# Manta-Network/Plonk-Prototype

Hardware: AMD Instinct MI355X
Metric: bls12_381_fr_ntt_butterflies_per_s (higher is better)
Workload: dtype u32x9 (29-bit limbs, Fr); 1 GPU; forward + inverse BLS12-381 Fr NTT, 2^20 points, device resident, natural order in/out, bit-exact vs oracle; log_n=20, parallelism=1 independent polynomial(s), one per GPU

## Files before the change

### include/plonk_mi355x.h

```cpp
#ifndef PLONK_MI355X_H
#define PLONK_MI355X_H

#include <stddef.h>
#include <stdint.h>

#ifdef __cplusplus
extern "C" {
#endif

typedef struct pm_ctx pm_ctx;
typedef struct pm_bases pm_bases;

typedef enum {
  PM_OK = 0,
  PM_ERR_BAD_ARG = -1,
  PM_ERR_DOMAIN_TOO_LARGE = -2,
  PM_ERR_OOM = -3,
  PM_ERR_HIP = -4,
  PM_ERR_NO_DEVICE = -5,
  PM_ERR_LENGTH = -6,
  PM_ERR_EXCHANGE = -7,
  PM_ERR_BUSY = -8,
  PM_ERR_POINT = -9
} pm_status;
// ... 411 lines not shown
int pm_profile_select(pm_ctx* ctx, const char* kernel_name);
int pm_profile_read(pm_ctx* ctx, char* buf, size_t cap);
int pm_test_field_op(pm_ctx* ctx, int op, const uint64_t* a, const uint64_t* b, uint64_t* out,
                     size_t n);
int pm_test_field_raw_op(pm_ctx* ctx, int field, int op, const uint32_t* in, uint32_t* out, size_t n);
int pm_test_g1_raw_op(pm_ctx* ctx, int op, const uint32_t* a, const uint32_t* b, uint32_t* out, size_t n);
int pm_test_glv_split(pm_ctx* ctx, const uint64_t* scalars, size_t n, uint32_t scalar_form, uint64_t* out);
int pm_test_host_glv_split(const uint64_t k[4], uint64_t out[4]);
int pm_test_jubjub_scalar_op(pm_ctx* ctx, int op, const uint64_t* a, const uint64_t* b, const uint64_t* c, uint64_t* out, size_t n);
int pm_test_host_jubjub_scalar_op(int op, const uint64_t* a, const uint64_t* b, const uint64_t* c, uint64_t* out, size_t n);
int pm_test_schnorr_stride(pm_ctx* ctx, size_t* stride);
int pm_test_cipher_stride(pm_ctx* ctx, size_t* stride);
int pm_test_cipher_digits(const uint64_t view_key[4], uint32_t scalar_form, int8_t digits[64]);
int pm_test_jubjub_msm_plan(size_t n, uint32_t batch, long window_bits, uint32_t num_cus, uint64_t out[8]);
int pm_test_jubjub_msm_digits(const uint64_t scalar[4], uint32_t c, int32_t* digits, uint32_t* n_digits);
int pm_test_host_field_op(int op, const uint64_t* a, const uint64_t* b, uint64_t* out, size_t n);
int pm_test_msm_sizing(size_t n, uint32_t batch, long window_bits, uint32_t table_window_bits, uint32_t num_cus,
                       uint64_t out[4]);
int pm_test_msm_plan(size_t n, uint32_t batch, long window_bits, uint32_t table_window_bits, uint32_t num_cus, long chunk,
                     long lb, uint32_t out[32], uint32_t* level_len);
int pm_test_ntt_plan(uint32_t log_n, uint32_t batch, long tile_log, long max_radix, long radix, uint32_t num_cus,
                     uint32_t out[20]);
int pm_test_ntt_step4_table(pm_ctx* ctx, uint32_t inverse, uint32_t S, uint32_t* out, size_t max_words, size_t* words);
int pm_test_ntt_exchange_map(uint32_t S, uint32_t LT, uint32_t ufast, uint32_t step, uint32_t tid, uint32_t out[12]);
int pm_test_wire_sort_plan(size_t n, size_t num_vars, uint32_t* passes, uint32_t* tiles, size_t* scratch_bytes);
int pm_test_host_naf(const uint64_t s[4], uint32_t rounds, int8_t* digits_msb_first, int* too_long);
int pm_test_msm_geometry(size_t n, long window_bits, uint32_t table_window_bits, uint32_t batch, uint32_t out[16],
                         uint32_t* part_of_bucket, uint32_t* first_bucket, uint32_t* width_bits);
int pm_test_plonk_linearise(size_t n, const uint64_t (*evaluations)[4], const uint64_t (*extras)[4],
                            const uint64_t (*challenges)[4], uint32_t selector_present_mask, uint64_t (*out_coeffs)[4],
                            uint32_t* out_roles, uint32_t* out_count, uint64_t out_r_z[4]);

#ifdef __cplusplus
}
#endif
#endif
```

### plonk-prototype_amd/_lib.py

```python
from __future__ import annotations

import ctypes as C
import os

_HERE = os.path.dirname(os.path.abspath(__file__))
LIB_PATH = os.environ.get("PM_LIB_PATH") or os.path.join(_HERE, "lib", "libplonk_mi355x.so")

u64p = C.POINTER(C.c_uint64)
u32p = C.POINTER(C.c_uint32)



class PermArgs(C.Structure):
    _fields_ = [("wires", C.c_void_p * 4), ("sigmas", C.c_void_p * 4), ("roots", C.c_void_p),
                ("beta", C.c_uint64 * 4), ("gamma", C.c_uint64 * 4), ("k", (C.c_uint64 * 4) * 3)]


class QuotientArgs(C.Structure):
    _fields_ = [("wires", C.c_void_p * 4), ("z", C.c_void_p), ("q_m", C.c_void_p), ("q_l", C.c_void_p),
                ("q_r", C.c_void_p), ("q_o", C.c_void_p), ("q_4", C.c_void_p), ("q_c", C.c_void_p),
                ("pi", C.c_void_p), ("sigmas", C.c_void_p * 4), ("l1", C.c_void_p), ("x", C.c_void_p),
                ("alpha", C.c_uint64 * 4), ("beta", C.c_uint64 * 4), ("gamma", C.c_uint64 * 4),
                ("k", (C.c_uint64 * 4) * 3), ("zh_inv", (C.c_uint64 * 4) * 4),
                ("q_arith", C.c_void_p), ("q_range", C.c_void_p), ("q_logic", C.c_void_p),
# ... 235 lines not shown
    "pm_test_comm_deadline": (C.c_int, [C.c_long, C.c_int, C.POINTER(C.c_int), C.POINTER(C.c_long), C.POINTER(C.c_int),
                                        C.POINTER(C.c_int), C.c_char_p, C.c_size_t]),
    "pm_keccak_f1600": (None, [C.c_char_p]),
    "pm_ntt_plan": (C.c_int, [C.c_uint32, u32p, u32p]),
    "pm_set_option": (C.c_int, [C.c_void_p, C.c_char_p, C.c_long]),
    "pm_profile_enable": (C.c_int, [C.c_void_p, C.c_int]),
    "pm_profile_select": (C.c_int, [C.c_void_p, C.c_char_p]),
    "pm_profile_read": (C.c_int, [C.c_void_p, C.c_char_p, C.c_size_t]),
    "pm_test_field_op": (C.c_int, [C.c_void_p, C.c_int, u64p, u64p, u64p, C.c_size_t]),
    "pm_test_field_raw_op": (C.c_int, [C.c_void_p, C.c_int, C.c_int, u32p, u32p, C.c_size_t]),
    "pm_test_g1_raw_op": (C.c_int, [C.c_void_p, C.c_int, u32p, u32p, u32p, C.c_size_t]),
    "pm_test_glv_split": (C.c_int, [C.c_void_p, u64p, C.c_size_t, C.c_uint32, u64p]),
    "pm_test_host_glv_split": (C.c_int, [u64p, u64p]),
    "pm_test_jubjub_scalar_op": (C.c_int, [C.c_void_p, C.c_int, u64p, u64p, u64p, u64p, C.c_size_t]),
    "pm_test_host_jubjub_scalar_op": (C.c_int, [C.c_int, u64p, u64p, u64p, u64p, C.c_size_t]),
    "pm_test_schnorr_stride": (C.c_int, [C.c_void_p, C.POINTER(C.c_size_t)]),
    "pm_test_cipher_stride": (C.c_int, [C.c_void_p, C.POINTER(C.c_size_t)]),
    "pm_test_cipher_digits": (C.c_int, [u64p, C.c_uint32, C.POINTER(C.c_int8)]),
    "pm_test_jubjub_msm_plan": (C.c_int, [C.c_size_t, C.c_uint32, C.c_long, C.c_uint32, u64p]),
    "pm_test_jubjub_msm_digits": (C.c_int, [u64p, C.c_uint32, C.POINTER(C.c_int32), u32p]),
    "pm_test_ntt_plan": (C.c_int, [C.c_uint32, C.c_uint32, C.c_long, C.c_long, C.c_long, C.c_uint32, C.POINTER(C.c_uint32)]),
    "pm_test_ntt_exchange_map": (C.c_int, [C.c_uint32] * 5 + [C.POINTER(C.c_uint32)]),
    "pm_test_ntt_step4_table": (C.c_int, [C.c_void_p, C.c_uint32, C.c_uint32, u32p, C.c_size_t, C.POINTER(C.c_size_t)]),
    "pm_test_wire_sort_plan": (C.c_int, [C.c_size_t, C.c_size_t, u32p, u32p, C.POINTER(C.c_size_t)]),
    "pm_test_host_naf": (C.c_int, [u64p, C.c_uint32, C.POINTER(C.c_int8), C.POINTER(C.c_int)]),
    "pm_test_msm_sizing": (C.c_int, [C.c_size_t, C.c_uint32, C.c_long, C.c_uint32, C.c_uint32, u64p]),
    "pm_test_msm_plan": (C.c_int, [C.c_size_t, C.c_uint32, C.c_long, C.c_uint32, C.c_uint32, C.c_long, C.c_long,
                                   u32p, u32p]),
    "pm_test_msm_geometry": (C.c_int, [C.c_size_t, C.c_long, C.c_uint32, C.c_uint32, C.POINTER(C.c_uint32),
                                      C.POINTER(C.c_uint32), C.POINTER(C.c_uint32), C.POINTER(C.c_uint32)]),
    "pm_test_plonk_linearise": (C.c_int, [C.c_size_t, u64p, u64p, u64p, C.c_uint32, u64p, u32p, u32p, u64p]),
}

PM_OK = 0
PM_ERR_BAD_ARG = -1
PM_ERR_DOMAIN_TOO_LARGE = -2
PM_ERR_OOM = -3
PM_ERR_HIP = -4
PM_ERR_NO_DEVICE = -5
PM_ERR_LENGTH = -6
PM_ERR_EXCHANGE = -7
PM_ERR_BUSY = -8
PM_ERR_POINT = -9

G1_CHECK_SUBGROUP = 1
G1_POINTS_IN_SUBGROUP = 1
# ... 78 lines not shown
```

### plonk-prototype_amd/csrc/api.hip

```cpp
#include <hip/hip_runtime.h>

#include <cstdio>
#include <cstdlib>
#include <cstring>

#include "context.h"
#include "field_inv.hip.h"
#include "fields.hip.h"
#include "host_field.h"
#include "jubjub_msm_plan.h"

namespace pm {

int set_err(pm_ctx* ctx, int code, const std::string& msg) {
  if (ctx) ctx->err = msg;
  return code;
}

int raise_lds_limit(pm_ctx* ctx, const void* fn, size_t bytes) {
  static std::mutex mu;
  static std::map<std::pair<int, const void*>, size_t> limit;
  std::lock_guard<std::mutex> lock(mu);
  size_t& have = limit[{ctx->device, fn}];
  if (bytes <= have) return PM_OK;
// ... 101 lines not shown
  int count = 0;
  if (hipGetDeviceCount(&count) != hipSuccess || count <= 0 || device_id < 0 || device_id >= count)
    return PM_ERR_NO_DEVICE;
  hipDeviceProp_t prop;
  if (hipGetDeviceProperties(&prop, device_id) != hipSuccess) return PM_ERR_NO_DEVICE;
  if (strncmp(prop.gcnArchName, "gfx950", 6) != 0) return PM_ERR_NO_DEVICE;
  if (hipSetDevice(device_id) != hipSuccess) return PM_ERR_HIP;
  pm_ctx* ctx = new pm_ctx();
  ctx->device = device_id;
  ctx->marks_on = getenv("PM_HOST_MARKS") != nullptr;
  ctx->num_cus = prop.multiProcessorCount;
  if (hipStreamCreateWithFlags(&ctx->stream, hipStreamNonBlocking) != hipSuccess) {
    delete ctx;
    return PM_ERR_HIP;
  }
  *out = ctx;
  return PM_OK;
}

static void release_caches(pm_ctx* ctx, bool all) {
  for (int d = 0; d < 2; ++d) {
    for (auto& kv : ctx->step_tw[d]) (void)hipFree(kv.second);
    for (auto& kv : ctx->step4_tw[d]) (void)hipFree(kv.second);
    for (auto& kv : ctx->domain[d]) {
      (void)hipFree(kv.second.tw_hi);
      (void)hipFree(kv.second.tw_lo);
      (void)hipFree(kv.second.cs_hi);
      (void)hipFree(kv.second.cs_lo);
      for (void* t : kv.second.pass_tw) (void)hipFree(t);
    }
    ctx->step_tw[d].clear();
    ctx->step4_tw[d].clear();
    ctx->domain[d].clear();
  }
  for (DeviceBuffer* b : {&ctx->ntt_tmp[0], &ctx->ntt_tmp[1], &ctx->io_in, &ctx->io_out, &ctx->msm_ws, &ctx->msm_scalars,
                          &ctx->poly_ws, &ctx->poly_tab, &ctx->jj_msm_ws, &ctx->fr_sqrt_tab}) {
    if (b->ptr) (void)hipFree(b->ptr);
    b->ptr = nullptr;
    b->bytes = 0;
  }
  if (all && ctx->msm_ctl.ptr) (void)hipFree(ctx->msm_ctl.ptr);
}

extern "C" int pm_trim(pm_ctx* ctx, size_t* freed_bytes) {
  if (!ctx) return PM_ERR_BAD_ARG;
  std::lock_guard<std::mutex> lk(ctx->mu);
  if (ctx->calls_holding_tables > 0)
    return set_err(ctx, PM_ERR_BUSY, "pm_trim while a pm_fr_ntt_fourstep_dev call is in flight on this context");
  PM_HIP(ctx, hipSetDevice(ctx->device));
  PM_HIP(ctx, hipDeviceSynchronize());
  size_t free0 = 0, free1 = 0, total = 0;
  PM_HIP(ctx, hipMemGetInfo(&free0, &total));
  release_caches(ctx, false);
  PM_HIP(ctx, hipMemGetInfo(&free1, &total));
  if (freed_bytes) *freed_bytes = free1 > free0 ? free1 - free0 : 0;
// ... 240 lines not shown
```

### plonk-prototype_amd/csrc/context.h

```cpp
#pragma once
#include <hip/hip_runtime.h>

#include <cstdint>
#include <initializer_list>
#include <map>
#include <chrono>
#include <mutex>
#include <string>
#include <vector>

#include "../../include/plonk_mi355x.h"

#ifndef PM_NTT_STEP_PRIO_DEFAULT
#define PM_NTT_STEP_PRIO_DEFAULT 1
#endif

namespace pm {

class ExchangeWatch;
void exchange_watch_free(ExchangeWatch* w);

struct DeviceBuffer {
  void* ptr = nullptr;
  size_t bytes = 0;
// ... 6 lines not shown
  hipEvent_t ev = nullptr;
};

struct NttDomainTables {
  void* tw_hi = nullptr;
  void* tw_lo = nullptr;
  void* cs_hi = nullptr;
  void* cs_lo = nullptr;
  void* pass_tw[4] = {nullptr, nullptr, nullptr, nullptr};
  unsigned pass_tw_key[4] = {0, 0, 0, 0};
  unsigned lh = 0;
};

}

struct pm_ctx {
  int device = 0;
  hipStream_t stream = nullptr;
  hipStream_t copy_in = nullptr, copy_out = nullptr;
  std::mutex mu;
  std::string err;
  std::map<unsigned, void*> step_tw[2];
  std::map<unsigned, void*> step4_tw[2];
  std::map<unsigned, pm::NttDomainTables> domain[2];
  pm::DeviceBuffer ntt_tmp[2];
  pm::DeviceBuffer io_in, io_out;
  pm::StreamOrder ord_ntt, ord_msm, ord_poly;
  bool marks_on = false;
  std::vector<std::pair<const char*, double>> marks;
  unsigned long long stat_alltoall_calls = 0, stat_alltoall_bytes = 0, stat_allgather_calls = 0, stat_transpose_steps = 0;
  int calls_holding_tables = 0;
  pm::DeviceBuffer msm_ws;
  pm::DeviceBuffer msm_ctl;
  unsigned msm_ctl_cap = 0;
  hipStream_t msm_side = nullptr;
  std::vector<hipEvent_t> msm_events;
  pm::DeviceBuffer msm_scalars;
  pm::DeviceBuffer jj_msm_ws;
  pm::StreamOrder ord_jj_msm;
  pm::DeviceBuffer fr_sqrt_tab;
  pm::DeviceBuffer poly_ws;
  pm::DeviceBuffer poly_tab;
  void* msm_host_pinned = nullptr;
  void* poly_host_pinned = nullptr;
  size_t msm_host_pinned_bytes = 0;
  void* comm = nullptr;
// ... 252 lines not shown
```

### plonk-prototype_amd/csrc/fields.hip.h

```cpp
#pragma once
#include <hip/hip_runtime.h>
#include <stdint.h>

namespace pm {

typedef uint32_t u32;
typedef unsigned long long u64;

#define PM_DEV __device__ __forceinline__
#define PM_HD __host__ __device__ constexpr

struct FrP {
  static constexpr int W = 29;
  static constexpr int N = 9;
  static constexpr int NS = 8;
  static constexpr u32 SAT[8] = {0x00000001u, 0xffffffffu, 0xfffe5bfeu, 0x53bda402u,
                                 0x09a1d805u, 0x3339d808u, 0x299d7d48u, 0x73eda753u};
};
struct FpP {
  static constexpr int W = 28;
  static constexpr int N = 14;
  static constexpr int NS = 12;
  static constexpr u32 SAT[12] = {0xffffaaabu, 0xb9feffffu, 0xb153ffffu, 0x1eabfffeu,
                                  0xf6b0f624u, 0x6730d2a0u, 0xf38512bfu, 0x64774b84u,
// ... 207 lines not shown
PM_DEV void fe_col_sqr(int k, u64& acc, const Fe<P>& a, const u32 (&d)[P::N], u32& tok) {
  constexpr int N = P::N;
#pragma unroll
  for (int i = 0; i < N; ++i) {
    const int j = k - i;
    if (j < 0 || j >= N || i > j) continue;
    fe_mac(acc, a.l[i], (i == j) ? a.l[i] : d[j], tok);
  }
}

template <class P>
PM_DEV Fe<P> fe_mul(const Fe<P>& a, const Fe<P>& b) {
  Fe<P> t;
  Fe<P>* const out[1] = {&t};
  fe_mont_cols<P, 1>([&](int k, u64* acc, u32& tok) { fe_col_mul<P>(k, acc[0], a, b, tok); }, out);
  return t;
}
template <class P, int G, int D, class WL>
PM_DEV Fe<P> fe_mul_split(const Fe<P>& x, WL&& wl) {
  constexpr int N = P::N, W = P::W;
  constexpr u32 MASK = Consts<P>::MASK;
  constexpr Limbs<N> M = Consts<P>::mod_limbs();
  static_assert(M.v[0] == 1u, "fe_mul_split: the modulus must be 1 mod 2^W");
  static_assert(G >= 1 && G <= N && D == G + 1 && D <= N, "fe_mul_split: one digit more than the longest group");
  Fe<P> r;
  u32 q[D];
  u64 acc = 0;
  u32 tok;
  PM_KEEP_INIT(tok);
#pragma unroll
  for (int k = 0; k < D + N - 1; ++k) {
#pragma unroll
    for (int i = 0; i < N; ++i) {
      const int b = k - i % G;
      if (b < 0 || b >= N) continue;
      fe_mac(acc, x.l[i], wl(i / G, b), tok);
    }
#pragma unroll
    for (int i = 0; i < D; ++i) {
      const int l = k - i;
      if (l < 1 || l >= N) continue;
      fe_mac(acc, q[i], M.v[l], tok);
    }
    if (k < D) {
      q[k] = (0u - (u32)acc) & MASK;
      acc += (u64)MASK;
    } else {
// ... 265 lines not shown
```

### plonk-prototype_amd/csrc/ntt.hip

```cpp
#include <hip/hip_runtime.h>

#include <condition_variable>
#include <thread>

#include <algorithm>
#include <cstring>

#include "context.h"
#include "host_field.h"
#include "ntt_kernels.hip.h"

namespace pm {

using host::HFr;

typedef void (*pass_fn)(const NttPassArgs, const NttConsts);
enum Role { ROLE_SINGLE = 0, ROLE_FIRST = 1, ROLE_MIDDLE = 2, ROLE_LAST = 3 };
pass_fn find_pass4(int S, int LT, int role);
struct PassEntry {
  int S, LT, role;
  pass_fn fn;
};
#define PM_SINGLE(X) X(3, 0) X(4, 0) X(5, 0) X(6, 0) X(7, 0) X(8, 0) X(9, 0) X(10, 0)
#define PM_MULTI(X) \
// ... 4 lines not shown
#undef X
#define X(S, LT)                                                      \
  {S, LT, ROLE_FIRST, ntt_pass_kernel<S, LT, true, false, true>},     \
      {S, LT, ROLE_MIDDLE, ntt_pass_kernel<S, LT, false, true, true>}, \
      {S, LT, ROLE_LAST, ntt_pass_kernel<S, LT, false, true, false>},
        PM_MULTI(X)
#undef X
};
static pass_fn find_pass(int S, int LT, int role) {
  for (const PassEntry& e : kPassTable)
    if (e.S == S && e.LT == LT && e.role == role) return e.fn;
  return nullptr;
}

size_t pass4_lds(int S, int LT);
unsigned pass4_threads(int S, int LT);
bool pass4_tw_producer(int S, int LT, int role);
bool pass4_step_prio(int S, int LT, int role);
#ifdef PM_DEV_STAMPS
int ntt_stamps_arm(pm_ctx* ctx, hipStream_t st, int pass, size_t waves);
#endif
int build_step4_table(pm_ctx* ctx, void** out, const NttConsts& c, unsigned S, hipStream_t st);
size_t step4_table_bytes(unsigned S);

struct Plan {
  int npass = 0;
  int S[4] = {0, 0, 0, 0};
  int LT[4] = {0, 0, 0, 0};
};
static Plan make_plan(unsigned log_n, int tile_log, int max_radix = 10, int radix = 4, unsigned min_tiles = 256,
                      unsigned batch = 1) {
  Plan p;
  if (log_n < 3) return p;
  if (log_n <= 10) {
    p.npass = 1;
    p.S[0] = (int)log_n;
    return p;
  }
  p.npass = (int)((log_n + max_radix - 1) / max_radix);
  p.npass = std::min(p.npass, (int)log_n / 5);
  p.npass = std::min(p.npass, 4);
  int base = (int)log_n / p.npass, extra = (int)log_n % p.npass;
  for (int i = 0; i < p.npass; ++i) {
    p.S[i] = base + (i < extra ? 1 : 0);
    int lt = tile_log ? tile_log - p.S[i] : (p.S[i] >= 10 && radix == 4 ? 1 : std::max(10 - p.S[i], 2));
    if (p.S[i] < 8 && lt > 11 - p.S[i]) lt = 11 - p.S[i];
// ... 69 lines not shown

static int get_step4_table(pm_ctx* ctx, int dir, unsigned S, void** out, hipStream_t st) {
  auto it = ctx->step4_tw[dir].find(S);
  if (it != ctx->step4_tw[dir].end()) {
    *out = it->second;
    return PM_OK;
  }
  HFr wR = domain_gen(S);
  if (dir) wR = host::inv(wR, host::FR());
  HFr w4 = domain_gen(2);
  HFr w16 = domain_gen(4);
  if (dir) w4 = host::inv(w4, host::FR());
  if (dir) w16 = host::inv(w16, host::FR());
  NttConsts c;
  memset(&c, 0, sizeof c);
  to_limbs(c.w8[0], wR);
  to_limbs(c.w8[1], w4);
  to_limbs(c.w8[2], w16);
  to_limbs(c.one, host::one(host::FR()));
  void* d = nullptr;
  int rc = build_step4_table(ctx, &d, c, S, st);
  if (rc) return rc;
  ctx->step4_tw[dir][S] = d;
  *out = d;
  return PM_OK;
}

static int get_domain_tables(pm_ctx* ctx, int dir, unsigned log_n, bool need_coset,
                             NttDomainTables** out, hipStream_t st) {
  NttDomainTables& t = ctx->domain[dir][log_n];
  const host::Field<4>& F = host::FR();
  t.lh = (log_n + 1) / 2;
  const u32 n_lo = 1u << t.lh, n_hi = 1u << (log_n - t.lh);
  auto build_pair = [&](const HFr& base, void** lo_out, void** hi_out) -> int {
    void *lo = nullptr, *hi = nullptr;
    int rc = build_pow_table(ctx, &lo, base, host::one(F), n_lo, 1, st);
    if (!rc) rc = build_pow_table(ctx, &hi, base, host::one(F), n_hi, n_lo, st);
    if (rc) {
      if (lo) (void)hipFree(lo);
      if (hi) (void)hipFree(hi);
      return rc;
    }
    *lo_out = lo;
    *hi_out = hi;
    return PM_OK;
  };
// ... 130 lines not shown
  for (int i = 0; i < std::min(ntmp, 2); ++i) {
    rc = ensure_buffer(ctx, ctx->ntt_tmp[i], (size_t)batch * n * 36);
    if (rc) return rc;
  }
  const void* src = d_in;
  unsigned log_ns = 0;
  a.wide_total = (unsigned long long)batch * n;
  a.wide_glog = plan_wide_glog(plan);
  bool tw_applied = false;
  for (int i = 0; i < plan.npass; ++i) {
    const bool last = (i == plan.npass - 1);
    const int S = plan.S[i], LT = plan.LT[i];
    void* dst = (last && !(plan.npass == 1 && inplace)) ? d_out : ctx->ntt_tmp[i & 1].ptr;
    const int role = plan.npass == 1 ? ROLE_SINGLE : (i == 0 ? ROLE_FIRST : (last ? ROLE_LAST : ROLE_MIDDLE));
    const bool r4 = ctx->opt_ntt_radix == 4 && find_pass4(S, LT, role) != nullptr;
    pass_fn fn = r4 ? find_pass4(S, LT, role) : find_pass(S, LT, role);
    if (!fn) return set_err(ctx, PM_ERR_BAD_ARG, "no kernel for this pass shape");
    void* stw = nullptr;
    rc = r4 ? get_step4_table(ctx, dir, (unsigned)S, &stw, st) : get_step_table(ctx, dir, (unsigned)S, &stw, st);
    if (rc) return rc;
    a.in = src;
    a.out = dst;
    a.step_tw = (const u32x4*)stw;
    a.batch_stride_in = in_stride;
    a.batch_stride_out = (plan.npass == 1 && inplace) ? n : out_stride;
    a.in_len = (u32)in_len;
    a.log_ns = log_ns;
    u32 post_i = last ? post : 0u;
    a.pass_tw = nullptr;
    a.pass_tw_out = nullptr;
    u32 tw_flag = 0;
    if (tw_applied) {
      tw_flag = PASS_TW_APPLIED;
    } else if (i > 0 && direct_tw) {
      void* ptw = nullptr;
      rc = get_pass_tw(ctx, dt, i, last, dir, log_n, log_ns, S, a.wide_glog, kc, st, &ptw);
      if (rc) return rc;
      a.pass_tw = ptw;
      tw_flag = PASS_DIRECT_TW;
    }
    tw_applied = false;
    if (!last && direct_tw && ctx->opt_ntt_tw_producer && r4 && pass4_tw_producer(S, LT, role)) {
      const bool next_last = (i + 1 == plan.npass - 1);
      const int nS = plan.S[i + 1];
      if (find_pass4(nS, plan.LT[i + 1], next_last ? ROLE_LAST : ROLE_MIDDLE) != nullptr) {
        void* ptw = nullptr;
// ... 212 lines not shown
    const int S = plan.S[i], LT = plan.LT[i];
    const bool r4 = rdx == 4 && find_pass4(S, LT, role) != nullptr;
    out[1 + 4 * i] = (uint32_t)S;
    out[2 + 4 * i] = (uint32_t)LT;
    out[3 + 4 * i] = r4 ? pass4_threads(S, LT) : std::max(64u, (1u << (S + LT)) / 8);
    out[4 + 4 * i] = (uint32_t)(r4 ? pass4_lds(S, LT) : pass_lds_bytes(S, LT));
    if ((r4 ? find_pass4(S, LT, role) : find_pass(S, LT, role)) != nullptr) out[17] |= 1u << i;
  }
  out[18] = plan.npass ? plan_wide_glog(plan) : 0u;
  return PM_OK;
}

extern "C" int pm_test_ntt_step4_table(pm_ctx* ctx, uint32_t inverse, uint32_t S, uint32_t* out, size_t max_words,
                                       size_t* words) {
  if (!ctx || inverse > 1 || S < 2 || S > 10 || (!out && max_words)) return PM_ERR_BAD_ARG;
  std::lock_guard<std::mutex> lk(ctx->mu);
  PM_HIP(ctx, hipSetDevice(ctx->device));
  OrderScope order_scope(ctx, ctx->ord_ntt, ctx->stream);
  if (order_scope.rc) return order_scope.rc;
  void* tab = nullptr;
  int rc = get_step4_table(ctx, (int)inverse, S, &tab, ctx->stream);
  if (rc) return rc;
  const size_t total = step4_table_bytes(S) / 4;
  if (words) *words = total;
  const size_t n = std::min(total, max_words);
  if (n) PM_HIP(ctx, hipMemcpyAsync(out, tab, n * 4, hipMemcpyDeviceToHost, ctx->stream));
  PM_HIP(ctx, hipStreamSynchronize(ctx->stream));
  return PM_OK;
}

extern "C" int pm_domain_prepare(pm_ctx* ctx, uint32_t log_n) {
  if (!ctx) return PM_ERR_BAD_ARG;
  std::lock_guard<std::mutex> lk(ctx->mu);
  if (log_n >= host::FR_TWO_ADICITY)
    return set_err(ctx, PM_ERR_DOMAIN_TOO_LARGE, "log_n >= 32 (Fr two-adicity)");
  PM_HIP(ctx, hipSetDevice(ctx->device));
  if (log_n == 0) return PM_OK;
  OrderScope order_scope(ctx, ctx->ord_ntt, ctx->stream);
  if (order_scope.rc) return order_scope.rc;
  Plan plan = make_plan(log_n, (int)ctx->opt_ntt_tile_log, (int)ctx->opt_ntt_max_radix, (int)ctx->opt_ntt_radix,
                        (unsigned)ctx->num_cus, 1);
  const unsigned wide_glog = plan_wide_glog(plan);
  for (int dir = 0; dir < 2; ++dir) {
    NttDomainTables* dt;
    int rc = get_domain_tables(ctx, dir, log_n, true, &dt, ctx->stream);
    if (rc) return rc;
    NttConsts kc;
    fill_consts(kc, dir, log_n);
    unsigned log_ns = 0;
    for (int i = 0; i < plan.npass; ++i) {
      const bool last = (i == plan.npass - 1);
      const int role = plan.npass == 1 ? ROLE_SINGLE : (i == 0 ? ROLE_FIRST : (last ? ROLE_LAST : ROLE_MIDDLE));
      const bool r4 = ctx->opt_ntt_radix == 4 && find_pass4(plan.S[i], plan.LT[i], role) != nullptr;
      void* stw;
      rc = r4 ? get_step4_table(ctx, dir, (unsigned)plan.S[i], &stw, ctx->stream)
              : get_step_table(ctx, dir, (unsigned)plan.S[i], &stw, ctx->stream);
      if (rc) return rc;
      if (i > 0 && log_n <= 26 && ctx->opt_ntt_direct_tw) {
        void* ptw;
        rc = get_pass_tw(ctx, dt, i, last, dir, log_n, log_ns, plan.S[i], wide_glog, kc, ctx->stream, &ptw);
        if (rc) return rc;
      }
      log_ns += (unsigned)plan.S[i];
    }
  }
  PM_HIP(ctx, hipStreamSynchronize(ctx->stream));
  return PM_OK;
}

extern "C" int pm_fr_ntt_dev(pm_ctx* ctx, const void* d_in, size_t in_len, size_t in_stride,
                             void* d_out, size_t out_stride, uint32_t log_n, uint32_t batch,
                             uint32_t flags, void* hip_stream) {
  if (!ctx) return PM_ERR_BAD_ARG;
  std::lock_guard<std::mutex> lk(ctx->mu);
  if (!d_out || (!d_in && in_len)) return set_err(ctx, PM_ERR_BAD_ARG, "null device pointer");
  hipStream_t st = hip_stream ? (hipStream_t)hip_stream : ctx->stream;
  return ntt_run(ctx, d_in, in_len, in_stride, d_out, out_stride, log_n, batch, flags, st);
}

extern "C" int pm_fr_ntt_batch(pm_ctx* ctx, const uint64_t* in, size_t in_len, size_t in_stride,
// ... 311 lines not shown
```

### plonk-prototype_amd/csrc/ntt4.hip

```cpp
#include <hip/hip_runtime.h>

#include <algorithm>

#include "context.h"
#include "ntt_kernels4.hip.h"

namespace pm {

typedef void (*pass_fn)(const NttPassArgs, const NttConsts);
struct Pass4Entry {
  int S, LT, role;
  pass_fn fn;
};
#define PM4_SINGLE(X) X(2, 0) X(3, 0) X(4, 0) X(5, 0) X(6, 0) X(7, 0) X(8, 0) X(9, 0) X(10, 0)
#define PM4_MULTI(X) X(5, 6) X(6, 5) X(7, 4) X(8, 3) X(9, 2) X(10, 1) X(10, 2) X(5, 5) X(6, 4) X(7, 3) X(8, 2) X(10, 0) X(9, 1)
static const Pass4Entry kPass4Table[] = {
#define X(S, LT) {S, LT, 0, ntt_pass4_kernel<S, LT, false, false, false>},
    PM4_SINGLE(X)
#undef X
#define X(S, LT)                                               \
  {S, LT, 1, ntt_pass4_kernel<S, LT, true, false, true>},      \
      {S, LT, 2, ntt_pass4_kernel<S, LT, false, true, true>},  \
      {S, LT, 3, ntt_pass4_kernel<S, LT, false, true, false>},
        PM4_MULTI(X)
#undef X
};

pass_fn find_pass4(int S, int LT, int role) {
  for (const Pass4Entry& e : kPass4Table)
    if (e.S == S && e.LT == LT && e.role == role) return e.fn;
  return nullptr;
}
bool pass4_tw_producer(int S, int LT, int role) {
  return (role == 1 || role == 2) && find_pass4(S, LT, role) != nullptr && step4_tw_producer(S, LT, role == 1, role == 2);
}
bool pass4_step_prio(int S, int LT, int role) { return find_pass4(S, LT, role) != nullptr && step4_has_prio(S); }
size_t pass4_lds(int S, int LT) { return pass4_lds_bytes(S, LT); }

#ifdef PM_DEV_STAMPS
static unsigned long long* g_host_stamps = nullptr;
static size_t g_host_stamp_waves = 0;
int ntt_stamps_arm(pm_ctx* ctx, hipStream_t st, int pass, size_t waves) {
  unsigned long long* p = nullptr;
  unsigned long long room = 0;
  if (g_host_stamps && (size_t)(pass + 1) * waves <= g_host_stamp_waves) {
    p = g_host_stamps + (size_t)pass * waves * NTT_STAMP_WORDS;
    room = waves;
  }
  PM_HIP(ctx, hipMemcpyToSymbolAsync(HIP_SYMBOL(g_ntt_stamps), &p, sizeof p, 0, hipMemcpyHostToDevice, st));
  PM_HIP(ctx, hipMemcpyToSymbolAsync(HIP_SYMBOL(g_ntt_stamp_waves), &room, sizeof room, 0, hipMemcpyHostToDevice, st));
  return PM_OK;
}
#endif
unsigned pass4_threads(int S, int LT) { return std::max(64u, (1u << (S + LT)) / 4); }

size_t step4_table_bytes(unsigned S) {
  return ((size_t)STEP4_HEAD + (size_t)step4_tw_total((int)S) * STEP4_ENTRY) * sizeof(u32x4);
}

int build_step4_table(pm_ctx* ctx, void** out, const NttConsts& c, unsigned S, hipStream_t st) {
  const u32 total = (u32)step4_tw_total((int)S);
  PM_HIP(ctx, hipMalloc(out, step4_table_bytes(S)));
  hipLaunchKernelGGL(step4_tw_kernel, dim3((std::max(total, 9u * STEP4_HEAD_CONSTS) + 255) / 256), dim3(256), 0, st,
                     (u32x4*)*out, c, S);
  PM_HIP(ctx, hipGetLastError());
  return PM_OK;
}

}

#ifdef PM_DEV_STAMPS
extern "C" int pm_dev_ntt_stamps(void* d_buf, size_t waves) {
  pm::g_host_stamps = (unsigned long long*)d_buf;
  pm::g_host_stamp_waves = d_buf ? waves : 0;
  return 0;
}
#endif
```

### plonk-prototype_amd/csrc/ntt_kernels.hip.h

```cpp
#pragma once
#include "fields.hip.h"

namespace pm {

struct NttConsts {
  u32 w8[3][9];
  u32 one[9];
  u32 scale[9];
};

struct NttPassArgs {
  const void* in;
  void* out;
  const u32x4* step_tw;
  const u32x4* tw_hi;
  const u32x4* tw_lo;
  const u32x4* cs_hi;
  const u32x4* cs_lo;
  const void* pass_tw;
  const void* pass_tw_out;
  unsigned long long batch_stride_in;
  unsigned long long batch_stride_out;
  unsigned long long wide_total;
  u32 wide_glog;
  u32 in_len;
  u32 log_n;
  u32 log_ns;
  u32 lh;
  u32 flags;
};
enum : u32 {
  PASS_DIRECT_TW = 1u,
  PASS_PRE_COSET = 2u,
  PASS_POST_SCALE = 4u,
  PASS_POST_COSET = 8u,
  PASS_XCD_REMAP = 16u,
  PASS_TW_OUT = 32u,
  PASS_TW_APPLIED = 64u,
  PASS_STEP_PRIO = 128u,
};

PM_DEV u32 xcd_tile(u32 b, u32 nb, u32 flags) {
  if (!(flags & PASS_XCD_REMAP) || (nb & 7u)) return b;
  return (b & 7u) * (nb >> 3) + (b >> 3);
}

PM_DEV Fr ld_tw(const u32x4* tab, size_t idx) {
  const u32x4* p = tab + 3 * idx;
  u32x4 a = p[0], b = p[1];
  u32 c = reinterpret_cast<const u32*>(p + 2)[0];
  Fr r;
  r.l[0] = a.x; r.l[1] = a.y; r.l[2] = a.z; r.l[3] = a.w;
// ... 361 lines not shown
```

### plonk-prototype_amd/csrc/ntt_kernels4.hip.h

```cpp
#pragma once
#include "ntt_kernels.hip.h"

namespace pm {

__host__ __device__ constexpr int step4_radix_log(int S, int s) { return (S - 2 * s) >= 2 ? 2 : 1; }
__host__ __device__ constexpr int num_steps4(int S) { return (S + 1) / 2; }
__host__ __device__ constexpr bool step4_plane_major(int S, bool in_wide) { return !in_wide && S >= 4 && S % 2 == 0; }
__host__ __device__ constexpr int step4_tw_offset(int S, int s) {
  int off = 0;
  for (int i = 0; i < s; ++i) off += ((1 << step4_radix_log(S, i)) - 1) << (2 * i);
  return off;
}
__host__ __device__ constexpr int step4_tw_total(int S) { return step4_tw_offset(S, num_steps4(S)); }
__host__ __device__ constexpr size_t pass4_lds_bytes(int S, int LT) {
  return num_steps4(S) > 1 ? ((size_t)36 << (S + LT)) : 0;
}

constexpr int STEP4_HEAD_CONSTS = 7;
constexpr int STEP4_HEAD_BLOCK = 84;
constexpr int STEP4_HEAD = STEP4_HEAD_CONSTS * STEP4_HEAD_BLOCK / 4;
constexpr int STEP4_ENTRY = 5;
__host__ __device__ constexpr int step4_head_exp(int blk) { return blk == 0 ? 4 : blk == 4 ? 6 : blk == 5 ? 9 : blk == 6 ? 0 : blk; }
typedef const __attribute__((address_space(4))) u32* W4Rows;
PM_DEV W4Rows w4_rows(const u32x4* step_tw) {
// ... 65 lines not shown
}

struct FrSplit2 {
  u32 l[18];
};
PM_DEV FrSplit2 ld_tw2(const u32x4* ent, size_t idx) {
  const u32x4* p = ent + STEP4_ENTRY * idx;
  u32x4 a = p[0], b = p[1], c = p[2], d = p[3];
  const uint2 e = reinterpret_cast<const uint2*>(p + 4)[0];
  FrSplit2 r;
  r.l[0] = a.x; r.l[1] = a.y; r.l[2] = a.z; r.l[3] = a.w;
  r.l[4] = b.x; r.l[5] = b.y; r.l[6] = b.z; r.l[7] = b.w;
  r.l[8] = c.x; r.l[9] = c.y; r.l[10] = c.z; r.l[11] = c.w;
  r.l[12] = d.x; r.l[13] = d.y; r.l[14] = d.z; r.l[15] = d.w;
  r.l[16] = e.x; r.l[17] = e.y;
  return r;
}
PM_DEV Fr mul_tw2(const Fr& x, const FrSplit2& w) {
  return fe_mul_split<FrP, 5, 6>(x, [&](int j, int b) { return w.l[9 * j + b]; });
}
__host__ __device__ constexpr bool step4_has_prio(int S) { return S >= 10 && num_steps4(S) >= 2; }
__host__ __device__ constexpr int step4_prio(int S, int s) { return num_steps4(S) - 1 - s < 3 ? num_steps4(S) - 1 - s : 3; }

#ifdef PM_DEV_STAMPS
constexpr int NTT_STAMP_WORDS = 40;
static __device__ unsigned long long* g_ntt_stamps = nullptr;
static __device__ unsigned long long g_ntt_stamp_waves = 0;
PM_DEV unsigned long long* ntt_stamp_slot() {
  const unsigned long long w =
      ((unsigned long long)blockIdx.y * gridDim.x + blockIdx.x) * ((blockDim.x + 63u) >> 6) + (threadIdx.x >> 6);
  return (g_ntt_stamps && w < g_ntt_stamp_waves && (threadIdx.x & 63u) == 0) ? g_ntt_stamps + w * NTT_STAMP_WORDS : nullptr;
}
PM_DEV void ntt_stamp(int k) {
  __builtin_amdgcn_sched_barrier(0);
  unsigned long long t, r;
  asm volatile("s_memtime %0\n\ts_memrealtime %1\n\ts_waitcnt lgkmcnt(0)" : "=&s"(t), "=&s"(r) : : "memory");
  if (unsigned long long* p = ntt_stamp_slot()) {
    p[2 * k] = t;
    p[2 * k + 1] = r;
  }
  __builtin_amdgcn_sched_barrier(0);
}
PM_DEV void ntt_stamp_placement() {
  const unsigned long long hw = __builtin_amdgcn_s_getreg(4 | (31 << 11));
  const unsigned long long xcc = __builtin_amdgcn_s_getreg(20 | (31 << 11));
  if (unsigned long long* p = ntt_stamp_slot()) {
    p[36] = hw | (xcc << 32);
    p[37] = (unsigned long long)blockIdx.x | ((unsigned long long)(threadIdx.x >> 6) << 32) | ((unsigned long long)blockIdx.y << 48);
  }
}
#define NTT_STAMP(k) ntt_stamp(k)
#define NTT_STAMP_LOADS(k)                          \
  do {                                              \
    asm volatile("s_waitcnt vmcnt(0)" ::: "memory"); \
    ntt_stamp(k);                                   \
  } while (0)
#else
#define NTT_STAMP(k)
#define NTT_STAMP_LOADS(k)
#endif

PM_DEV void dft4s(Fr& a0, Fr& a1, Fr& a2, Fr& a3, W4Rows w4) {
  BFLY(3, a0, a2);
  BFLY(3, a1, a3);
  a3 = mul_head(a3, w4);
  a2 = fe_norm<FrP>(a2);
  BFLY(5, a0, a1);
  BFLY(3, a2, a3);
  Fr t = a1;
  a1 = a2;
  a2 = t;
}

template <int S, int LT, bool OUT_UFAST>
PM_DEV size_t pass4_out_index(const NttPassArgs& a, u32 tid, size_t j0, int m) {
  constexpr int R = 1 << S;
  constexpr int U = R / 4;
  const u32 c = OUT_UFAST ? tid / U : tid & ((1u << LT) - 1u);
  const u32 u = OUT_UFAST ? tid % U : tid >> LT;
  const size_t j = j0 + c;
  const size_t ns = (size_t)1 << a.log_ns;
  const size_t k = j & (ns - 1);
  return (j - k) * R + k + (size_t)(u + m * U) * ns;
}

template <int S, int LT, int STEP, bool OUT_UFAST, bool IN_WIDE, bool OUT_WIDE>
PM_DEV void ntt_step4(Fr (&x)[4], Fr (&ptw)[4], const NttPassArgs& a, const NttConsts& kc, u32x4* lds0, u32x4* lds1,
                      u32* lds2, W4Rows w4, u32 tid, size_t j0) {
  constexpr int R = 1 << S;
  constexpr int T = 1 << LT;
  constexpr int U = R / 4;
  constexpr int NSTEPS = num_steps4(S);
  constexpr int LQ = step4_radix_log(S, STEP);
  constexpr u32 nsp = 1u << (2 * STEP);
  constexpr bool last = (STEP == NSTEPS - 1);
  constexpr bool ufast = OUT_UFAST && last;
  constexpr bool L1_UNIFORM = step4_l1_uniform(S, LT, IN_WIDE);
  constexpr bool PM = step4_plane_major(S, IN_WIDE);
  constexpr bool L1_CONSUMER = PM && step4_l1_consumer(S, LT, OUT_UFAST);
  constexpr bool TW_PRODUCER = OUT_WIDE && step4_tw_producer(S, LT, OUT_UFAST, IN_WIDE);
  static_assert(!(L1_UNIFORM && STEP == 0 && ufast), "the producer of the first-layer twiddles is in wave order");
  const u32 c = ufast ? tid / U : tid & (T - 1);
  const u32 u = ufast ? tid % U : tid >> LT;
  constexpr int PRIO = step4_prio(S, STEP);
  if constexpr (step4_has_prio(S) && STEP > 0 && PRIO != step4_prio(S, STEP - 1)) {
    if (a.flags & PASS_STEP_PRIO) __builtin_amdgcn_s_setprio(PRIO);
  }
  if (STEP > 0) {
#pragma unroll
    for (int m = 0; m < 4; ++m) {
      const u32 e = PM ? step4_pm_read(S, LT, OUT_UFAST, STEP, tid, m) : (u + m * U) * T + c;
      u32x4 lo = lds0[e], hi = lds1[e];
      x[m].l[0] = lo.x; x[m].l[1] = lo.y; x[m].l[2] = lo.z; x[m].l[3] = lo.w;
      x[m].l[4] = hi.x; x[m].l[5] = hi.y; x[m].l[6] = hi.z; x[m].l[7] = hi.w;
      x[m].l[8] = lds2[e];
    }
  }
  NTT_STAMP(2 + 3 * STEP);
  const u32x4* stw = a.step_tw + STEP4_HEAD + STEP4_ENTRY * step4_tw_offset(S, STEP);
  if constexpr (LQ == 2) {
    const u32 kp = PM ? step4_pm_digit(S, STEP, u) : u & (nsp - 1);
    if constexpr (L1_CONSUMER && STEP == 1) {
      const u32 ku = __builtin_amdgcn_readfirstlane(kp);
      x[0] = fe_reduce_weak<FrP>(x[0]);
#pragma unroll
      for (int m = 1; m < 4; ++m) {
        W4Rows rows = w16_rows(w4, ku * m);
        asm volatile("" : "+s"(rows));
        x[m] = mul_head(x[m], rows);
      }
    } else if (STEP > 0 && !(L1_UNIFORM && STEP == 1)) {
      x[0] = fe_reduce_weak<FrP>(x[0]);
      x[1] = mul_tw2(x[1], ld_tw2(stw, 0 * nsp + kp));
      x[2] = mul_tw2(x[2], ld_tw2(stw, 1 * nsp + kp));
      const FrSplit2 w3 = ld_tw2(stw, 2 * nsp + kp);
      if constexpr (TW_PRODUCER && STEP >= NSTEPS - 2) {
        if (a.flags & PASS_TW_OUT) {
          const WidePtr wtw = wide_ptrs(const_cast<void*>(a.pass_tw_out), a.wide_glog);
          constexpr int m0 = last ? 2 : 0;
          __builtin_amdgcn_sched_barrier(0);
          ptw[m0] = ld_wide(wtw, pass4_out_index<S, LT, OUT_UFAST>(a, tid, j0, m0));
          ptw[m0 + 1] = ld_wide(wtw, pass4_out_index<S, LT, OUT_UFAST>(a, tid, j0, m0 + 1));
          __builtin_amdgcn_sched_barrier(0);
        }
      }
      x[3] = mul_tw2(x[3], w3);
    }
    W4Rows w4s = w4;
    asm volatile("" : "+s"(w4s));
    dft4s(x[0], x[1], x[2], x[3], w4s);
    if constexpr (L1_UNIFORM && STEP == 0) {
      const u32 m = __builtin_amdgcn_readfirstlane(u >> (S - 4));
      x[0] = fe_reduce_weak<FrP>(x[0]);
#pragma unroll
      for (int t = 1; t < 4; ++t) {
        W4Rows rows = w16_rows(w4, t * m);
        asm volatile("" : "+s"(rows));
        x[t] = mul_head(x[t], rows);
      }
    }
    NTT_STAMP(2 + 3 * STEP + 1);
    if constexpr (!last) {
      __syncthreads();
      const u32 base = (u - kp) * 4 + kp;
#pragma unroll
      for (int t = 0; t < 4; ++t) {
        const u32 e = PM ? step4_pm_write(S, LT, OUT_UFAST, STEP, tid, t) : (base + t * nsp) * T + c;
        lds0[e] = u32x4{x[t].l[0], x[t].l[1], x[t].l[2], x[t].l[3]};
        lds1[e] = u32x4{x[t].l[4], x[t].l[5], x[t].l[6], x[t].l[7]};
        lds2[e] = x[t].l[8];
      }
      __syncthreads();
      NTT_STAMP(2 + 3 * STEP + 2);
// ... 143 lines not shown
  u32 off = 0;
  for (u32 s = 0; 2 * s < S; ++s) {
    const u32 lq = (S - 2 * s) >= 2 ? 2 : 1;
    const u32 nsp = 1u << (2 * s);
    const u32 cnt = ((1u << lq) - 1) * nsp;
    if (i >= off && i < off + cnt) {
      const u32 t = (i - off) / nsp + 1, kp = (i - off) % nsp;
      const u32 e = (kp * t) << (S - 2 * s - lq);
      const Fr w = fr_pow(fr_limbs(c.w8[0]), e, fr_limbs(c.one));
      const Fr r0 = fr_canon(fe_mul<FrP>(w, fe_pow2<FrP, 174>()));
      const Fr r1 = fr_canon(fe_mul<FrP>(w, fe_pow2<FrP, 319>()));
      u32x4* p = ent + STEP4_ENTRY * (size_t)i;
      p[0] = u32x4{r0.l[0], r0.l[1], r0.l[2], r0.l[3]};
      p[1] = u32x4{r0.l[4], r0.l[5], r0.l[6], r0.l[7]};
      p[2] = u32x4{r0.l[8], r1.l[0], r1.l[1], r1.l[2]};
      p[3] = u32x4{r1.l[3], r1.l[4], r1.l[5], r1.l[6]};
      p[4] = u32x4{r1.l[7], r1.l[8], 0u, 0u};
      return;
    }
    off += cnt;
  }
}

}
```

Before: 130.2 billion butterflies/s.

## Add lazy-reduction twiddle tables and DFT4 for S=10 LT=1 radix-4 passes

Adds a second precomputed twiddle table with G-grouped split rows, used for the S=10, LT=1 radix-4 pass configuration. In those passes it uses a lazy split Montgomery multiply (D == G digits) and a lazy DFT4 variant. The goal is to cut the number of reduction digits and the arithmetic per twiddle multiply, at the cost of wider table entries to load and looser output bounds, with larger butterfly bound parameters to match. The fe_mul_split static assert is relaxed to allow D == G.

```diff
diff --git a/include/plonk_mi355x.h b/include/plonk_mi355x.h
--- a/include/plonk_mi355x.h
+++ b/include/plonk_mi355x.h
@@ -457,6 +457,8 @@
 int pm_test_ntt_plan(uint32_t log_n, uint32_t batch, long tile_log, long max_radix, long radix, uint32_t num_cus,
                      uint32_t out[20]);
 int pm_test_ntt_step4_table(pm_ctx* ctx, uint32_t inverse, uint32_t S, uint32_t* out, size_t max_words, size_t* words);
+int pm_test_ntt_step4_lazy_table(pm_ctx* ctx, uint32_t inverse, uint32_t S, uint32_t G, uint32_t* out, size_t max_words,
+                                 size_t* words);
 int pm_test_ntt_exchange_map(uint32_t S, uint32_t LT, uint32_t ufast, uint32_t step, uint32_t tid, uint32_t out[12]);
 int pm_test_wire_sort_plan(size_t n, size_t num_vars, uint32_t* passes, uint32_t* tiles, size_t* scratch_bytes);
 int pm_test_host_naf(const uint64_t s[4], uint32_t rounds, int8_t* digits_msb_first, int* too_long);
diff --git a/plonk-prototype_amd/_lib.py b/plonk-prototype_amd/_lib.py
--- a/plonk-prototype_amd/_lib.py
+++ b/plonk-prototype_amd/_lib.py
@@ -281,6 +281,8 @@
     "pm_test_ntt_plan": (C.c_int, [C.c_uint32, C.c_uint32, C.c_long, C.c_long, C.c_long, C.c_uint32, C.POINTER(C.c_uint32)]),
     "pm_test_ntt_exchange_map": (C.c_int, [C.c_uint32] * 5 + [C.POINTER(C.c_uint32)]),
     "pm_test_ntt_step4_table": (C.c_int, [C.c_void_p, C.c_uint32, C.c_uint32, u32p, C.c_size_t, C.POINTER(C.c_size_t)]),
+    "pm_test_ntt_step4_lazy_table": (C.c_int, [C.c_void_p, C.c_uint32, C.c_uint32, C.c_uint32, u32p, C.c_size_t,
+                                               C.POINTER(C.c_size_t)]),
     "pm_test_wire_sort_plan": (C.c_int, [C.c_size_t, C.c_size_t, u32p, u32p, C.POINTER(C.c_size_t)]),
     "pm_test_host_naf": (C.c_int, [u64p, C.c_uint32, C.POINTER(C.c_int8), C.POINTER(C.c_int)]),
     "pm_test_msm_sizing": (C.c_int, [C.c_size_t, C.c_uint32, C.c_long, C.c_uint32, C.c_uint32, u64p]),
diff --git a/plonk-prototype_amd/csrc/api.hip b/plonk-prototype_amd/csrc/api.hip
--- a/plonk-prototype_amd/csrc/api.hip
+++ b/plonk-prototype_amd/csrc/api.hip
@@ -147,6 +147,7 @@
   for (int d = 0; d < 2; ++d) {
     for (auto& kv : ctx->step_tw[d]) (void)hipFree(kv.second);
     for (auto& kv : ctx->step4_tw[d]) (void)hipFree(kv.second);
+    for (auto& kv : ctx->step4_lazy_tw[d]) (void)hipFree(kv.second);
     for (auto& kv : ctx->domain[d]) {
       (void)hipFree(kv.second.tw_hi);
       (void)hipFree(kv.second.tw_lo);
@@ -156,6 +157,7 @@
     }
     ctx->step_tw[d].clear();
     ctx->step4_tw[d].clear();
+    ctx->step4_lazy_tw[d].clear();
     ctx->domain[d].clear();
   }
   for (DeviceBuffer* b : {&ctx->ntt_tmp[0], &ctx->ntt_tmp[1], &ctx->io_in, &ctx->io_out, &ctx->msm_ws, &ctx->msm_scalars,
diff --git a/plonk-prototype_amd/csrc/context.h b/plonk-prototype_amd/csrc/context.h
--- a/plonk-prototype_amd/csrc/context.h
+++ b/plonk-prototype_amd/csrc/context.h
@@ -52,6 +52,7 @@
   std::string err;
   std::map<unsigned, void*> step_tw[2];
   std::map<unsigned, void*> step4_tw[2];
+  std::map<unsigned, void*> step4_lazy_tw[2];
   std::map<unsigned, pm::NttDomainTables> domain[2];
   pm::DeviceBuffer ntt_tmp[2];
   pm::DeviceBuffer io_in, io_out;
diff --git a/plonk-prototype_amd/csrc/fields.hip.h b/plonk-prototype_amd/csrc/fields.hip.h
--- a/plonk-prototype_amd/csrc/fields.hip.h
+++ b/plonk-prototype_amd/csrc/fields.hip.h
@@ -253,7 +253,8 @@
   constexpr u32 MASK = Consts<P>::MASK;
   constexpr Limbs<N> M = Consts<P>::mod_limbs();
   static_assert(M.v[0] == 1u, "fe_mul_split: the modulus must be 1 mod 2^W");
-  static_assert(G >= 1 && G <= N && D == G + 1 && D <= N, "fe_mul_split: one digit more than the longest group");
+  static_assert(G >= 1 && G <= N && (D == G + 1 || D == G) && D <= N,
+                "fe_mul_split: one digit more than the longest group, or as many (lazy: the value stays above 2 m)");
   Fe<P> r;
   u32 q[D];
   u64 acc = 0;
diff --git a/plonk-prototype_amd/csrc/ntt.hip b/plonk-prototype_amd/csrc/ntt.hip
--- a/plonk-prototype_amd/csrc/ntt.hip
+++ b/plonk-prototype_amd/csrc/ntt.hip
@@ -50,6 +50,9 @@
 #endif
 int build_step4_table(pm_ctx* ctx, void** out, const NttConsts& c, unsigned S, hipStream_t st);
 size_t step4_table_bytes(unsigned S);
+int pass4_lazy_form(int S, int LT, int role);
+int build_step4_lazy_table(pm_ctx* ctx, void** out, const NttConsts& c, unsigned S, unsigned G, hipStream_t st);
+size_t step4_lazy_table_bytes(unsigned S, unsigned G);
 
 struct Plan {
   int npass = 0;
@@ -165,6 +168,30 @@
   int rc = build_step4_table(ctx, &d, c, S, st);
   if (rc) return rc;
   ctx->step4_tw[dir][S] = d;
+  *out = d;
+  return PM_OK;
+}
+
+static int get_step4_lazy_table(pm_ctx* ctx, int dir, unsigned S, unsigned G, void** out, hipStream_t st) {
+  const unsigned key = S << 8 | G;
+  auto it = ctx->step4_lazy_tw[dir].find(key);
+  if (it != ctx->step4_lazy_tw[dir].end()) {
+    *out = it->second;
+    return PM_OK;
+  }
+  HFr wR = domain_gen(S);
+  HFr w4 = domain_gen(2);
+  if (dir) wR = host::inv(wR, host::FR());
+  if (dir) w4 = host::inv(w4, host::FR());
+  NttConsts c;
+  memset(&c, 0, sizeof c);
+  to_limbs(c.w8[0], wR);
+  to_limbs(c.w8[1], w4);
+  to_limbs(c.one, host::one(host::FR()));
+  void* d = nullptr;
+  int rc = build_step4_lazy_table(ctx, &d, c, S, G, st);
+  if (rc) return rc;
+  ctx->step4_lazy_tw[dir][key] = d;
   *out = d;
   return PM_OK;
 }
@@ -341,6 +368,13 @@
     a.in = src;
     a.out = dst;
     a.step_tw = (const u32x4*)stw;
+    a.step_tw_lazy = nullptr;
+    if (const int lazy = r4 ? pass4_lazy_form(S, LT, role) : 0) {
+      void* ltw = nullptr;
+      rc = get_step4_lazy_table(ctx, dir, (unsigned)S, (unsigned)lazy, &ltw, st);
+      if (rc) return rc;
+      a.step_tw_lazy = (const u32x4*)ltw;
+    }
     a.batch_stride_in = in_stride;
     a.batch_stride_out = (plan.npass == 1 && inplace) ? n : out_stride;
     a.in_len = (u32)in_len;
@@ -599,6 +633,24 @@
   int rc = get_step4_table(ctx, (int)inverse, S, &tab, ctx->stream);
   if (rc) return rc;
   const size_t total = step4_table_bytes(S) / 4;
+  if (words) *words = total;
+  const size_t n = std::min(total, max_words);
+  if (n) PM_HIP(ctx, hipMemcpyAsync(out, tab, n * 4, hipMemcpyDeviceToHost, ctx->stream));
+  PM_HIP(ctx, hipStreamSynchronize(ctx->stream));
+  return PM_OK;
+}
+
+extern "C" int pm_test_ntt_step4_lazy_table(pm_ctx* ctx, uint32_t inverse, uint32_t S, uint32_t G, uint32_t* out,
+                                            size_t max_words, size_t* words) {
+  if (!ctx || inverse > 1 || S < 2 || S > 10 || !(G == 1 || G == 2 || G == 3 || G == 5) || (!out && max_words)) return PM_ERR_BAD_ARG;
+  std::lock_guard<std::mutex> lk(ctx->mu);
+  PM_HIP(ctx, hipSetDevice(ctx->device));
+  OrderScope order_scope(ctx, ctx->ord_ntt, ctx->stream);
+  if (order_scope.rc) return order_scope.rc;
+  void* tab = nullptr;
+  int rc = get_step4_lazy_table(ctx, (int)inverse, S, G, &tab, ctx->stream);
+  if (rc) return rc;
+  const size_t total = step4_lazy_table_bytes(S, G) / 4;
   if (words) *words = total;
   const size_t n = std::min(total, max_words);
   if (n) PM_HIP(ctx, hipMemcpyAsync(out, tab, n * 4, hipMemcpyDeviceToHost, ctx->stream));
@@ -633,6 +685,10 @@
       rc = r4 ? get_step4_table(ctx, dir, (unsigned)plan.S[i], &stw, ctx->stream)
               : get_step_table(ctx, dir, (unsigned)plan.S[i], &stw, ctx->stream);
       if (rc) return rc;
+      if (const int lazy = r4 ? pass4_lazy_form(plan.S[i], plan.LT[i], role) : 0) {
+        rc = get_step4_lazy_table(ctx, dir, (unsigned)plan.S[i], (unsigned)lazy, &stw, ctx->stream);
+        if (rc) return rc;
+      }
       if (i > 0 && log_n <= 26 && ctx->opt_ntt_direct_tw) {
         void* ptw;
         rc = get_pass_tw(ctx, dt, i, last, dir, log_n, log_ns, plan.S[i], wide_glog, kc, ctx->stream, &ptw);
diff --git a/plonk-prototype_amd/csrc/ntt4.hip b/plonk-prototype_amd/csrc/ntt4.hip
--- a/plonk-prototype_amd/csrc/ntt4.hip
+++ b/plonk-prototype_amd/csrc/ntt4.hip
@@ -35,6 +35,9 @@
   return (role == 1 || role == 2) && find_pass4(S, LT, role) != nullptr && step4_tw_producer(S, LT, role == 1, role == 2);
 }
 bool pass4_step_prio(int S, int LT, int role) { return find_pass4(S, LT, role) != nullptr && step4_has_prio(S); }
+int pass4_lazy_form(int S, int LT, int role) {
+  return find_pass4(S, LT, role) != nullptr ? step4_lazy_form(S, LT, role == 2 || role == 3) : 0;
+}
 size_t pass4_lds(int S, int LT) { return pass4_lds_bytes(S, LT); }
 
 #ifdef PM_DEV_STAMPS
@@ -67,6 +70,18 @@
   return PM_OK;
 }
 
+size_t step4_lazy_table_bytes(unsigned S, unsigned G) {
+  return ((size_t)STEP4_LAZY_HEAD + (size_t)step4_lazy_total((int)S) * step4_lazy_entry((int)G)) * sizeof(u32x4);
+}
+
+int build_step4_lazy_table(pm_ctx* ctx, void** out, const NttConsts& c, unsigned S, unsigned G, hipStream_t st) {
+  const u32 total = (u32)step4_lazy_total((int)S);
+  PM_HIP(ctx, hipMalloc(out, step4_lazy_table_bytes(S, G)));
+  hipLaunchKernelGGL(step4_lazy_tw_kernel, dim3((std::max(total, 9u) + 255) / 256), dim3(256), 0, st, (u32x4*)*out, c, S, G);
+  PM_HIP(ctx, hipGetLastError());
+  return PM_OK;
+}
+
 }
 
 #ifdef PM_DEV_STAMPS
diff --git a/plonk-prototype_amd/csrc/ntt_kernels.hip.h b/plonk-prototype_amd/csrc/ntt_kernels.hip.h
--- a/plonk-prototype_amd/csrc/ntt_kernels.hip.h
+++ b/plonk-prototype_amd/csrc/ntt_kernels.hip.h
@@ -28,6 +28,7 @@
   u32 log_ns;
   u32 lh;
   u32 flags;
+  const u32x4* step_tw_lazy;
 };
 enum : u32 {
   PASS_DIRECT_TW = 1u,
diff --git a/plonk-prototype_amd/csrc/ntt_kernels4.hip.h b/plonk-prototype_amd/csrc/ntt_kernels4.hip.h
--- a/plonk-prototype_amd/csrc/ntt_kernels4.hip.h
+++ b/plonk-prototype_amd/csrc/ntt_kernels4.hip.h
@@ -111,6 +111,52 @@
 __host__ __device__ constexpr bool step4_has_prio(int S) { return S >= 10 && num_steps4(S) >= 2; }
 __host__ __device__ constexpr int step4_prio(int S, int s) { return num_steps4(S) - 1 - s < 3 ? num_steps4(S) - 1 - s : 3; }
 
+__host__ __device__ constexpr int step4_lazy_form(int S, int LT, bool in_wide) {
+  return S == 10 && LT == 1 ? (in_wide ? 3 : 5) : 0;
+}
+constexpr int STEP4_LAZY_HEAD = STEP4_HEAD_BLOCK / 4;
+__host__ __device__ constexpr int step4_lazy_rows(int G) { return (9 + G - 1) / G; }
+__host__ __device__ constexpr int step4_lazy_entry(int G) { return (9 * step4_lazy_rows(G) + 3) / 4; }
+__host__ __device__ constexpr bool step4_lazy_step(int S, int s) { return s >= 2 && s < num_steps4(S) && step4_radix_log(S, s) == 2; }
+__host__ __device__ constexpr int step4_lazy_offset(int S, int s) {
+  int off = 0;
+  for (int i = 2; i < s; ++i) off += step4_lazy_step(S, i) ? 3 << (2 * i) : 0;
+  return off;
+}
+__host__ __device__ constexpr int step4_lazy_total(int S) { return step4_lazy_offset(S, num_steps4(S)); }
+
+template <int G>
+struct FrSplitLazy {
+  u32 l[9 * step4_lazy_rows(G)];
+};
+template <int G>
+PM_DEV FrSplitLazy<G> ld_tw_lazy(const u32x4* ent, size_t idx) {
+  constexpr int WORDS = 9 * step4_lazy_rows(G), UNITS = step4_lazy_entry(G);
+  const u32x4* p = ent + UNITS * idx;
+  FrSplitLazy<G> r;
+#pragma unroll
+  for (int k = 0; k < UNITS; ++k) {
+    if (WORDS - 4 * k == 2) {
+      const uint2 e = reinterpret_cast<const uint2*>(p + k)[0];
+      r.l[4 * k] = e.x; r.l[4 * k + 1] = e.y;
+    } else {
+      const u32x4 v = p[k];
+      r.l[4 * k] = v.x;
+      if (4 * k + 1 < WORDS) r.l[4 * k + 1] = v.y;
+      if (4 * k + 2 < WORDS) r.l[4 * k + 2] = v.z;
+      if (4 * k + 3 < WORDS) r.l[4 * k + 3] = v.w;
+    }
+  }
+  return r;
+}
+template <int G>
+PM_DEV Fr mul_tw_lazy(const Fr& x, const FrSplitLazy<G>& w) {
+  return fe_mul_split<FrP, G, G>(x, [&](int j, int b) { return w.l[9 * j + b]; });
+}
+PM_DEV Fr mul_head_lazy(const Fr& x, W4Rows rows) {
+  return fe_mul_split<FrP, 1, 1>(x, [&](int j, int b) { return rows[9 * b + j]; });
+}
+
 #ifdef PM_DEV_STAMPS
 constexpr int NTT_STAMP_WORDS = 40;
 static __device__ unsigned long long* g_ntt_stamps = nullptr;
@@ -156,6 +202,18 @@
   a2 = fe_norm<FrP>(a2);
   BFLY(5, a0, a1);
   BFLY(3, a2, a3);
+  Fr t = a1;
+  a1 = a2;
+  a2 = t;
+}
+
+PM_DEV void dft4s_lazy(Fr& a0, Fr& a1, Fr& a2, Fr& a3, W4Rows w4) {
+  BFLY(18, a0, a2);
+  BFLY(18, a1, a3);
+  a3 = mul_head_lazy(a3, w4);
+  a2 = fe_norm<FrP>(a2);
+  BFLY(34, a0, a1);
+  BFLY(39, a2, a3);
   Fr t = a1;
   a1 = a2;
   a2 = t;
@@ -188,7 +246,9 @@
   constexpr bool PM = step4_plane_major(S, IN_WIDE);
   constexpr bool L1_CONSUMER = PM && step4_l1_consumer(S, LT, OUT_UFAST);
   constexpr bool TW_PRODUCER = OUT_WIDE && step4_tw_producer(S, LT, OUT_UFAST, IN_WIDE);
+  constexpr int LAZY = step4_lazy_form(S, LT, IN_WIDE);
   static_assert(!(L1_UNIFORM && STEP == 0 && ufast), "the producer of the first-layer twiddles is in wave order");
+  static_assert(!LAZY || !step4_generic(S, LT, OUT_UFAST, IN_WIDE, STEP) || step4_lazy_step(S, STEP), "the lazy table starts at step 2");
   const u32 c = ufast ? tid / U : tid & (T - 1);
   const u32 u = ufast ? tid % U : tid >> LT;
   constexpr int PRIO = step4_prio(S, STEP);
@@ -207,6 +267,18 @@
   }
   NTT_STAMP(2 + 3 * STEP);
   const u32x4* stw = a.step_tw + STEP4_HEAD + STEP4_ENTRY * step4_tw_offset(S, STEP);
+  const auto ld_step = [&](size_t i) {
+    if constexpr (LAZY != 0)
+      return ld_tw_lazy<LAZY>(a.step_tw_lazy + STEP4_LAZY_HEAD + step4_lazy_entry(LAZY) * step4_lazy_offset(S, STEP), i);
+    else
+      return ld_tw2(stw, i);
+  };
+  const auto mul_step = [](const Fr& v, const auto& w) {
+    if constexpr (LAZY != 0)
+      return mul_tw_lazy<LAZY>(v, w);
+    else
+      return mul_tw2(v, w);
+  };
   if constexpr (LQ == 2) {
     const u32 kp = PM ? step4_pm_digit(S, STEP, u) : u & (nsp - 1);
     if constexpr (L1_CONSUMER && STEP == 1) {
@@ -220,9 +292,9 @@
       }
     } else if (STEP > 0 && !(L1_UNIFORM && STEP == 1)) {
       x[0] = fe_reduce_weak<FrP>(x[0]);
-      x[1] = mul_tw2(x[1], ld_tw2(stw, 0 * nsp + kp));
-      x[2] = mul_tw2(x[2], ld_tw2(stw, 1 * nsp + kp));
-      const FrSplit2 w3 = ld_tw2(stw, 2 * nsp + kp);
+      x[1] = mul_step(x[1], ld_step(0 * nsp + kp));
+      x[2] = mul_step(x[2], ld_step(1 * nsp + kp));
+      const auto w3 = ld_step(2 * nsp + kp);
       if constexpr (TW_PRODUCER && STEP >= NSTEPS - 2) {
         if (a.flags & PASS_TW_OUT) {
           const WidePtr wtw = wide_ptrs(const_cast<void*>(a.pass_tw_out), a.wide_glog);
@@ -233,11 +305,14 @@
           __builtin_amdgcn_sched_barrier(0);
         }
       }
-      x[3] = mul_tw2(x[3], w3);
-    }
-    W4Rows w4s = w4;
+      x[3] = mul_step(x[3], w3);
+    }
+    W4Rows w4s = LAZY != 0 ? w4_rows(a.step_tw_lazy) : w4;
     asm volatile("" : "+s"(w4s));
-    dft4s(x[0], x[1], x[2], x[3], w4s);
+    if constexpr (LAZY != 0)
+      dft4s_lazy(x[0], x[1], x[2], x[3], w4s);
+    else
+      dft4s(x[0], x[1], x[2], x[3], w4s);
     if constexpr (L1_UNIFORM && STEP == 0) {
       const u32 m = __builtin_amdgcn_readfirstlane(u >> (S - 4));
       x[0] = fe_reduce_weak<FrP>(x[0]);
@@ -427,4 +502,38 @@
   }
 }
 
-}
+static __global__ void step4_lazy_tw_kernel(u32x4* out, const NttConsts c, u32 S, u32 G) {
+  const u32 i = blockIdx.x * blockDim.x + threadIdx.x;
+  const auto pow29 = [](u32 e) {
+    Fr p = fe_pow2<FrP, 29>();
+    for (u32 k = 1; k < e; ++k) p = fe_mul<FrP>(p, fe_pow2<FrP, 261 + 29>());
+    return p;
+  };
+  if (i < 9) {
+    const Fr row = fr_canon(fe_mul<FrP>(fr_limbs(c.w8[1]), pow29(i + 1)));
+    u32* head = reinterpret_cast<u32*>(out);
+    for (u32 b = 0; b < 9; ++b) head[9 * b + i] = row.l[b];
+    if (i < 3) head[81 + i] = 0u;
+  }
+  const u32 rows = (9 + G - 1) / G, units = (9 * rows + 3) / 4;
+  u32 off = 0;
+  for (u32 s = 2; 2 * s + 2 <= S; ++s) {
+    const u32 nsp = 1u << (2 * s);
+    const u32 cnt = 3 * nsp;
+    if (i >= off && i < off + cnt) {
+      const u32 t = (i - off) / nsp + 1, kp = (i - off) % nsp;
+      const u32 e = (kp * t) << (S - 2 * s - 2);
+      const Fr w = fr_pow(fr_limbs(c.w8[0]), e, fr_limbs(c.one));
+      u32* p = reinterpret_cast<u32*>(out + STEP4_LAZY_HEAD + (size_t)units * i);
+      for (u32 j = 0; j < rows; ++j) {
+        const Fr row = fr_canon(fe_mul<FrP>(w, pow29(j * G + G)));
+        for (u32 b = 0; b < 9; ++b) p[9 * j + b] = row.l[b];
+      }
+      for (u32 k = 9 * rows; k < 4 * units; ++k) p[k] = 0u;
+      return;
+    }
+    off += cnt;
+  }
+}
+
+}
```

After: 133.3 billion butterflies/s (median of 6 runs). +2.4%, better.
